# tanishqkumar/ssd

Measured on AMD Instinct MI355X. Metric: output tokens/sec + p50 TTFT, Llama-3-70B SSD k=7 f=3; mean accepted len, higher is better.
Workload: dtype bf16

## Files before the change

ssd_amd/csrc/common.h:

```cpp
#pragma once
#include <hip/hip_runtime.h>
#include <stdint.h>
#include <stdlib.h>

typedef uint16_t bf16_t;
typedef __attribute__((ext_vector_type(8))) __bf16 bf16x8_t;
typedef __attribute__((ext_vector_type(4))) float f32x4_t;
typedef __attribute__((ext_vector_type(4))) short s16x4_t;
typedef __attribute__((ext_vector_type(4))) uint32_t u32x4_t;
typedef __attribute__((ext_vector_type(2))) uint32_t u32x2_t;
constexpr int SSD_MAX_DEVICES = 16;

#include "ssd_hip.h"
#include "ssd_hip_tune.h"
#include "ssd_hip_quant.h"
#include "ssd_hip_w4a16.h"
#include "ssd_hip_w4zp.h"
#include "ssd_hip_mxfp4.h"

__device__ __forceinline__ float bf2f(uint32_t bits16) { return __uint_as_float(bits16 << 16); }

__device__ __forceinline__ uint32_t f2bf(float f) {
  uint32_t u = __float_as_uint(f);
  if ((u & 0x7fffffffu) > 0x7f800000u) return (u >> 16) | 0x40u;
  u += 0x7fffu + ((u >> 16) & 1u);
  return u >> 16;
}
__device__ __forceinline__ uint32_t pack_bf2(float lo, float hi) { return f2bf(lo) | (f2bf(hi) << 16); }

typedef __attribute__((ext_vector_type(2))) float f32x2_t;
typedef __attribute__((ext_vector_type(2))) __bf16 bf16x2_t;
__device__ __forceinline__ uint32_t pack_bf2_hw(float lo, float hi) {
  return __builtin_bit_cast(uint32_t, __builtin_convertvector(f32x2_t{lo, hi}, bf16x2_t));
// ... 92 lines not shown
```

ssd_amd/csrc/gemm.hip:

```cpp
#include "common.h"

enum { EPI_ROWS = 0, EPI_SILU_FRAG = 1, EPI_ROWS_F32 = 2, EPI_ROWS_ARGMAX = 3 };

struct ArgPart { float v; int i; };
__device__ __forceinline__ ArgPart arg_better(ArgPart a, ArgPart b) {
  return (b.v > a.v || (b.v == a.v && b.i < a.i)) ? b : a;
}

extern "C" int ssd_gemm_splitk(const void* x_frag, const void* w_frag, const void* bias, void* y, int M, int N, int K, int ldy,
                               int splits, int waves, void* workspace, void* counters, void* stream);

template <int MT, int NT>
struct Stage {
  u32x4_t a[NT];
  u32x4_t b[MT];
};

template <int MT, int NT, int EPI, bool DEEP = false>
__global__ void __launch_bounds__(DEEP ? 512 : 1024)
gemm_wf_kernel(const u32x4_t* __restrict__ Wf, const u32x4_t* __restrict__ Xf,
               const bf16_t* __restrict__ bias, void* __restrict__ Yv, int M, int N, int K, int ldy, int tpw,
               float* __restrict__ part_val, int* __restrict__ part_idx, int part_stride) {
  extern __shared__ __attribute__((aligned(16))) char smem[];
  constexpr int KTS = EPI == EPI_SILU_FRAG ? 8 : 9;
  KTRACE(KTS, 0);
  const int lane = threadIdx.x & 63;
  const int wave = __builtin_amdgcn_readfirstlane(threadIdx.x >> 6);
  const int nw = blockDim.x >> 6;
  const int KT = K >> 5;
  const int ntiles = (N / 16) / NT;
  const int t_begin = blockIdx.x * tpw, t_end = min(ntiles, t_begin + tpw);
  const u32x4_t* xp = Xf + lane;
  const size_t wstride = (size_t)KT << 6;
  const size_t xstride = (size_t)KT << 6;
  constexpr int U = ((MT + NT <= 3) ? 4 : ((MT + NT <= 6) ? 2 : 1)) * (DEEP ? 2 : 1);
  Stage<MT, NT> cur[U], nxt[U];
  const int kstep = nw * U;
  const int kt0 = wave * U;
// ... 2 lines not shown
  const int mt_last = (M - 1) >> 4;
  auto load = [&](Stage<MT, NT>(&s)[U], int kt) {
#pragma unroll
    for (int u = 0; u < U; ++u) {
#pragma unroll
      for (int nt = 0; nt < NT; ++nt)
        s[u].a[nt] = __builtin_nontemporal_load(wp + nt * wstride + ((size_t)(kt + u) << 6));
#pragma unroll
      for (int mt = 0; mt < MT; ++mt) {
        u32x4_t b = {0u, 0u, 0u, 0u};
        if (NT > 1 || mt * 16 + (lane & 15) < M) b = xp[(mt < mt_last ? mt : mt_last) * xstride + ((size_t)(kt + u) << 6)];
        s[u].b[mt] = b;
      }
    }
  };
  if (t_begin < t_end && kt0 < kmain) load(cur, kt0);
  ArgPart run[MT];
#pragma unroll
  for (int mt = 0; mt < MT; ++mt) run[mt] = ArgPart{-INFINITY, 0x7fffffff};

  for (int tile = t_begin; tile < t_end; ++tile) {
  const int tile0 = tile * NT;
  f32x4_t acc[NT][MT];
#pragma unroll
  for (int nt = 0; nt < NT; ++nt)
#pragma unroll
    for (int mt = 0; mt < MT; ++mt) acc[nt][mt] = f32x4_t{0.f, 0.f, 0.f, 0.f};

  auto compute = [&](Stage<MT, NT>(&s)[U]) {
#pragma unroll
    for (int u = 0; u < U; ++u)
#pragma unroll
      for (int nt = 0; nt < NT; ++nt)
#pragma unroll
        for (int mt = 0; mt < MT; ++mt) acc[nt][mt] = mfma16(s[u].a[nt], s[u].b[mt], acc[nt][mt]);
  };

  int kt = kt0;
  if (kt < kmain) {
    for (; kt + kstep < kmain; kt += kstep) {
      load(nxt, kt + kstep);
      compute(cur);
#pragma unroll
      for (int u = 0; u < U; ++u) cur[u] = nxt[u];
    }
    compute(cur);
  }
  for (kt = (wave == nw - 1) ? kmain : KT; kt < KT; ++kt) {
#pragma unroll
    for (int nt = 0; nt < NT; ++nt) {
      u32x4_t a = __builtin_nontemporal_load(wp + nt * wstride + ((size_t)kt << 6));
#pragma unroll
      for (int mt = 0; mt < MT; ++mt) {
        u32x4_t b = {0u, 0u, 0u, 0u};
        if (mt * 16 + (lane & 15) < M) b = xp[mt * xstride + ((size_t)kt << 6)];
        acc[nt][mt] = mfma16(a, b, acc[nt][mt]);
// ... 102 lines not shown
static int launch_t(const void* x, const void* w, const void* bias, void* y, int M, int N, int K, int ldy,
                    int waves, int tpw, hipStream_t st, float* part_val = nullptr, int* part_idx = nullptr, int part_stride = 0) {
  const int ntiles = (N / 16) / NT;
  if (tpw < 1) tpw = 1;
  const int blocks = (ntiles + tpw - 1) / tpw;
  if (EPI == EPI_ROWS_ARGMAX && (!part_val || !part_idx || part_stride < blocks)) return SSD_ERR_ARG;
  size_t lds = (size_t)waves * NT * MT * 64 * sizeof(f32x4_t);
  if (EPI == EPI_ROWS_ARGMAX) lds += (size_t)waves * MT * 16 * sizeof(ArgPart);
  if (DEEP && waves > 8) return SSD_ERR_ARG;
  auto kern = gemm_wf_kernel<MT, NT, EPI, DEEP>;
  if (lds > 64 * 1024) {
    if (hipFuncSetAttribute(reinterpret_cast<const void*>(kern), hipFuncAttributeMaxDynamicSharedMemorySize, (int)lds) != hipSuccess)
      return SSD_ERR_LAUNCH;
  }
  hipLaunchKernelGGL(kern, dim3(blocks), dim3(waves * 64), lds, st, (const u32x4_t*)w, (const u32x4_t*)x,
                     (const bf16_t*)bias, y, M, N, K, ldy, tpw, part_val, part_idx, part_stride);
  return hipGetLastError() == hipSuccess ? SSD_OK : SSD_ERR_LAUNCH;
}

template <int MT, int EPI>
static int launch_nt(const void* x, const void* w, const void* bias, void* y, int M, int N, int K, int ldy,
                     int nt, int waves, int tpw, hipStream_t st) {
  if (nt == 1) {
    if constexpr (EPI == EPI_SILU_FRAG) return SSD_ERR_ARG;
    else return launch_t<MT, 1, EPI>(x, w, bias, y, M, N, K, ldy, waves, tpw, st);
  }
  if (nt == 2) return launch_t<MT, 2, EPI>(x, w, bias, y, M, N, K, ldy, waves, tpw, st);
  if (nt == 4) {
    if constexpr (MT > 2) return SSD_ERR_ARG;
    else return launch_t<MT, 4, EPI>(x, w, bias, y, M, N, K, ldy, waves, tpw, st);
  }
// ... 63 lines not shown
  }
  int nt = 1;
  if (epilogue == EPI_SILU_FRAG) nt = 2;
  else if (mt >= 4 && groups % 2 == 0) nt = 2;
  else if (groups >= 2048 && groups % 2 == 0) nt = 2;
  int waves = 16;
  while (waves > 1 && KT / waves < 4) waves >>= 1;
  const int blocks = groups / nt;
  if (blocks >= 1024 && waves > 8) waves = 8;
  if (mt == 2 && blocks >= 512 && blocks < 2048 && waves > 4 && KT / 4 >= 4) waves = 4;
  if (mt >= 4 && waves > 8) waves = 8;
  if (mt >= 8 && waves > 4) waves = 4;
  return ssd_gemm_wf_cfg(x_frag, w_frag, bias, y, M, N, K, ldy, epilogue, nt, waves, stream);
}


static void argmax_head_cfg(int M, int N, int K, int* nt, int* waves, int* tpw) {
  const int groups = N / 16, KT = K / 32;
  if (M <= 16) {
    ssd_pick_skinny_cfg(groups, KT, false, nt, waves, tpw);
    return;
  }
  int n = (groups >= 2048 && groups % 2 == 0) ? 2 : 1;
  int w = 16;
  while (w > 1 && KT / w < 4) w >>= 1;
  const int blocks = groups / n;
  if (blocks >= 1024 && w > 8) w = 8;
  if (blocks >= 512 && blocks < 2048 && w > 4 && KT / 4 >= 4) w = 4;
  *nt = n; *waves = w; *tpw = 1;
}
// ... 28 lines not shown
```

ssd_amd/csrc/gemm_fused.hip:

```cpp
#include "common.h"
#include <type_traits>

enum { FEPI_ROWS = 0, FEPI_SILU_FRAG = 1, FEPI_QKV_ROPE = 3 };

struct FusedParams {
  const u32x4_t* Wf;
  const u32x4_t* Xf;
  const bf16_t* h;
  const float* h_parts;
  int S;
  const bf16_t* res_in;
  bf16_t* res_out;
  const bf16_t* norm_w;
  const bf16_t* bias;
  void* y;
  const int64_t* positions;
  const float* cos_sin;
  const int32_t* slots;
  bf16_t* q_out;
  bf16_t* k_cache;
  bf16_t* v_cache;
  float eps;
  int M, N, K, ldy;
  int nh, nkv, hd, bs;
// ... 14 lines not shown
    }
#pragma unroll
    for (int j = 0; j < 4; ++j) { hf[j] = round_bf(lo[j]); hf[4 + j] = round_bf(hi[j]); }
  } else {
    const u32x4_t hv = *reinterpret_cast<const u32x4_t*>(p.h + (size_t)mm * p.K + k8 * 8);
#pragma unroll
    for (int j = 0; j < 4; ++j) { hf[2 * j] = bf2f(hv[j] & 0xffffu); hf[2 * j + 1] = bf2f(hv[j] >> 16); }
  }
#pragma unroll
  for (int j = 0; j < 4; ++j) {
    x[2 * j] = hf[2 * j] + bf2f(rv[j] & 0xffffu);
    x[2 * j + 1] = hf[2 * j + 1] + bf2f(rv[j] >> 16);
  }
}

template <int NT, int EPI, bool XNORM, int FUSED_MAXC>
__global__ void __launch_bounds__(1024) gemm_fused_kernel(const FusedParams p) {
  extern __shared__ __attribute__((aligned(16))) char smem[];
  constexpr int KTS = !XNORM ? 2 : (EPI == FEPI_QKV_ROPE ? 0 : 1);
  KTRACE(KTS, 0);
  const int lane = threadIdx.x & 63;
  const int wave = __builtin_amdgcn_readfirstlane(threadIdx.x >> 6);
  const int nw = blockDim.x >> 6;
  const int M = p.M, K = p.K;
  const int KT = K >> 5, K8 = K >> 3;
  const int tile0 = blockIdx.x * NT;
  const int mcol = lane & 15, q4 = lane >> 4;
  u32x4_t* xlds = reinterpret_cast<u32x4_t*>(smem + p.scratch_bytes);

  f32x4_t acc[NT];
#pragma unroll
  for (int nt = 0; nt < NT; ++nt) acc[nt] = f32x4_t{0.f, 0.f, 0.f, 0.f};
  const u32x4_t* wp = p.Wf + ((size_t)tile0 * KT << 6) + lane;
// ... 3 lines not shown
  u32x4_t wa[2][U][NT];
  u32x4_t xg[2][U];
  auto loadw = [&](int buf, int kt) {
#pragma unroll
    for (int u = 0; u < U; ++u) {
#pragma unroll
      for (int nt = 0; nt < NT; ++nt)
        wa[buf][u][nt] = __builtin_nontemporal_load(wp + nt * wstride + ((size_t)(kt + u) << 6));
      if (!XNORM) {
        u32x4_t b = {0u, 0u, 0u, 0u};
        if (mcol < M) b = p.Xf[((size_t)(kt + u) << 6) + lane];
        xg[buf][u] = b;
      }
    }
  };
  const int kstep = nw * U;
  const int kt0 = wave * U;
  const int ngroups = KT / U;
  const int nmain = ngroups > wave ? (ngroups - wave + nw - 1) / nw : 0;
  if (nmain > 0) loadw(0, kt0);
  if (nmain > 1) loadw(1, kt0 + kstep);
  float pre_cs[8];
  int pre_slot = -1;
  bool pre_ok = false;
  if (EPI == FEPI_QKV_ROPE && wave < NT && mcol < M) {
    const int grp = tile0 + wave;
    const int gph = p.hd >> 4;
    pre_slot = p.slots[mcol];
    if (grp < (p.nh + p.nkv) * gph) {
      const int d = (grp % gph) * 8 + (q4 & 1) * 4;
      const float* cs = p.cos_sin + (size_t)p.positions[mcol] * p.hd;
      const f32x4_t c4 = *reinterpret_cast<const f32x4_t*>(cs + d), s4 = *reinterpret_cast<const f32x4_t*>(cs + (p.hd >> 1) + d);
#pragma unroll
      for (int r = 0; r < 4; ++r) { pre_cs[r] = c4[r]; pre_cs[4 + r] = s4[r]; }
    }
    pre_ok = true;
  }
  KTRACE(KTS, 1);
  if (XNORM) {
    float* ssbuf = reinterpret_cast<float*>(smem);
    constexpr int MC = FUSED_MAXC > 0 ? FUSED_MAXC : 1;
    float x32[MC][8];
    u32x4_t wv[MC];
    const int total = M * K8;
    const bool cached = FUSED_MAXC > 0 && total <= FUSED_MAXC * (int)blockDim.x;
    const int cpb = (K8 + gridDim.x - 1) / gridDim.x;
    if (!cached) {
      for (int c = threadIdx.x; c < total; c += blockDim.x) {
        const int mm = c / K8, k8 = c % K8;
        float xx[8];
        fused_load_x32(p, mm, k8, xx);
        float ss = 0.f;
        u32x4_t o;
// ... 350 lines not shown
  FusedParams q = p;
  if (XNORM) {
    const size_t chunks = (size_t)p.M * (p.K / 8);
    const size_t need = chunks * 4 + (size_t)waves * 64;
    if (lds < need) lds = (need + 15) & ~(size_t)15;
    q.scratch_bytes = (int)lds;
    lds += chunks * 16;
    if (lds > 160 * 1024) return SSD_ERR_SHAPE;
  } else {
    q.scratch_bytes = (int)lds;
  }
  auto kern = gemm_fused_kernel<NT, EPI, XNORM, MAXC>;
  if (lds > 64 * 1024 &&
      hipFuncSetAttribute(reinterpret_cast<const void*>(kern), hipFuncAttributeMaxDynamicSharedMemorySize, (int)lds) != hipSuccess)
    return SSD_ERR_LAUNCH;
  hipLaunchKernelGGL(kern, dim3(blocks), dim3(waves * 64), lds, st, q);
  return hipGetLastError() == hipSuccess ? SSD_OK : SSD_ERR_LAUNCH;
}

template <int NT, int EPI, bool XNORM>
static int launch_fused(const FusedParams& p, int waves, hipStream_t st) {
  if constexpr (XNORM) {
    if (p.M * (p.K / 8) <= waves * 64) return launch_fused_c<NT, EPI, true, 1>(p, waves, st);
    return launch_fused_c<NT, EPI, true, 0>(p, waves, st);
  } else {
    return launch_fused_c<NT, EPI, false, 1>(p, waves, st);
  }
}

template <int EPI, bool XNORM>
static int launch_fused_nt(const FusedParams& p, int nt, int waves, hipStream_t st) {
// ... 61 lines not shown
                              const int32_t* slots, void* q_out, void* k_cache, void* v_cache, int nh, int nkv, int hd,
                              int block_size, int nt, int waves, void* stream) {
  return fused_impl(x_frag, h_rows, nullptr, 0, res_in, res_out, norm_w, eps, w_frag, bias, M, N, K, epilogue, y, ldy, positions,
                    cos_sin, slots, q_out, k_cache, v_cache, nh, nkv, hd, block_size, nt, waves, stream);
}

extern "C" int ssd_gemm_fused_parts(const void* h_parts, int splits, const void* res_in, void* res_out, const void* norm_w,
                                    float eps, const void* w_frag, const void* bias, int M, int N, int K, int epilogue, void* y,
                                    int ldy, const int64_t* positions, const float* cos_sin, const int32_t* slots, void* q_out,
                                    void* k_cache, void* v_cache, int nh, int nkv, int hd, int block_size, int nt, int waves,
                                    void* stream) {
  return fused_impl(nullptr, nullptr, (const float*)h_parts, splits, res_in, res_out, norm_w, eps, w_frag, bias, M, N, K, epilogue,
                    y, ldy, positions, cos_sin, slots, q_out, k_cache, v_cache, nh, nkv, hd, block_size, nt, waves, stream);
}

KT_DEFINE_SETTER(gemm_fused)
```

ssd_amd/engine/model_runner.py:

```python
from __future__ import annotations

import torch
import torch.distributed as dist

from ssd_amd.hip import ops as H
from ssd_amd.hip.lib import load_library
from ssd_amd.model import HipDecoder, AttnMeta
from ssd_amd.model_config import ModelConfig
from ssd_amd import weights as W
from ssd_amd.utils.graphs import capture
from ssd_amd.engine.async_proto import to_device


class ModelRunner:
    PREFILL_GRAPHS = 4
    PREFILL_GRAPH_MAX_T = 1024

    def __init__(self, config, model_cfg: ModelConfig, *, is_draft: bool, device: torch.device, tp_rank: int = 0,
                 tp_size: int = 1, tp_group=None, model_path: str | None = None, weights_seed: int = 0,
                 gen_device: str | None = None, num_kvcache_blocks: int = -1, memory_utilization: float | None = None,
                 max_decode_tokens: int | None = None, weight_source=None, force_collectives: bool = False,
                 custom_ar: bool | None = None):
        if not torch.cuda.is_available():
            raise RuntimeError("ssd_amd.ModelRunner needs an MI355X; there is no CPU fallback on the product path")
# ... 137 lines not shown
        self.sx = self.config.sampler_x
        self.sx_k = (self.config.async_fan_out + 1) if self.sx is not None else 0
        if self.sx is not None:
            rows = max(B * K, self.max_bs * getattr(self.config, "MQ_LEN", 1))
            self.d_boost = torch.zeros(rows, self.sx_k, dtype=torch.int32, **dev)

    def _check_collectives(self) -> None:
        ar = self.model.custom_ar
        if ar is not None and ar.failed():
            raise RuntimeError("one-shot all-reduce timed out waiting for a peer; results of this step are invalid "
                               "(rerun with SSD_CUSTOM_AR=0 to use RCCL)")
        if self._has_chain_err() and (int(self._chain_err_host[0]) or int(self.model.chain_err.item())):
            self._raise_chain_err()

    def _has_chain_err(self) -> bool:
        return getattr(self.model, "chain_seg", False) or getattr(self.model, "tree_seg", False)

    def _raise_chain_err(self):
        raise RuntimeError("a bounded wait inside a resident layer segment (csrc/chain.hip / csrc/tree_segment.hip) gave up; the draft "
                           "forwards since the last check are invalid (rerun with SSD_CHAIN_SEG=0 SSD_TREE_SEG=0 for the separate launches)")

    def _post_chain_err(self) -> None:
        if self._has_chain_err():
            self._chain_err_host.copy_(self.model.chain_err, non_blocking=True)

    def _check_chain_host(self) -> None:
        if self._has_chain_err() and int(self._chain_err_host[0]):
            self._raise_chain_err()

    def check_segments(self, sync: bool = False) -> None:
        if not self._has_chain_err():
            return
        if int(self._chain_err_host[0]) or (sync and int(self.model.chain_err.item())):
            self._raise_chain_err()

# ... 593 lines not shown
```

ssd_amd/model.py:

```python
from __future__ import annotations

from dataclasses import dataclass

import os

import torch
import torch.distributed as dist

from ssd_amd.hip import ops as H
from ssd_amd.hip import quant_ops as Q
from ssd_amd.hip import w4_ops as W4
from ssd_amd.hip import w4zp_ops as W4Z
from ssd_amd.hip import mx4_ops as MX4
from ssd_amd import quant
from ssd_amd.model_config import ModelConfig

BF16 = torch.bfloat16


@dataclass
class AttnMeta:
    mode: int
    B: int
    max_q: int
    slot_mapping: torch.Tensor
    context_lens: torch.Tensor
    block_tables: torch.Tensor
    cu_q: torch.Tensor | None = None
# ... 86 lines not shown
        _validated = _geo == (2048, 2048, 8192, 3072, 64)
        self.chain_seg = ((_cs == "1" or (_cs == "auto" and _validated)) and not cfg.qk_norm and tp_size == 1 and not self.use_coll and not self.quantized
                          and taps is None and H.chain_segment_ok(self.h, self.qn, self.I, self.qkv_n, self.nh, self.nkv, self.hd))
        _ts = os.environ.get("SSD_TREE_SEG", "auto")
        self.tree_seg_rows = 32 if _ts == "1" else 16
        self.tree_seg_colocated = False
        self.tree_seg = ((_ts == "1" or (_ts == "auto" and _validated)) and tp_size == 1 and not self.use_coll and not self.quantized
                         and taps is None and max_tokens >= 2
                         and H.tree_segment_ok(2, self.h, self.qn, self.I, self.qkv_n, self.nh, self.nkv, self.hd))
        if self.chain_seg:
            self.chain_gr = z(H.chain_granule_bytes(self.h, self.I) // 8, dtype=torch.int64)
            self.buf_res3 = z(1, self.h)
        if self.chain_seg or self.tree_seg:
            self.chain_gen = z(1, dtype=torch.int32)
            self.chain_err = z(1, dtype=torch.int32)
        if self.tree_seg:
            self.tree_ws = z(H.tree_segment_workspace_bytes(self.h, self.I) // 8, dtype=torch.int64)
            self.buf_res_b = z(min(T, 32), self.h)
        self._last_parts = False
        pt = min(T, 32)
        self.buf_parts_o = z(16 * pt * self.h, dtype=torch.float32) if self.use_parts else None
        self.buf_parts_d = z(16 * pt * self.h, dtype=torch.float32) if self.use_parts else None
        self.logits = z(self.max_logit_rows, self.V)
        self.taps = sorted(set(taps)) if taps else None
        self.acts = z(T, len(self.taps) * self.h) if self.taps else None
        self.max_splits = 16
        pf_shapes = [(self.qkv_n, self.h), (self.h, self.qn), (2 * self.I, self.h), (self.h, self.I), (self.V, self.h)]
        need = max([H.gemm_pf_workspace_bytes(128, n, k) // 4 for n, k in pf_shapes if self._pf_eligible(n, k)], default=0)
        self._lm_ok = max_tokens > 128
        if self._lm_ok:
# ... 380 lines not shown
                   parts: bool | None = None, pf_src: int = 0) -> None:
        cfg, w = self.cfg, self.w
        p = f"model.layers.{li}."
        small, norm_fuse = self.fusion_plan(T)
        kc, vc = self.kv_cache[li, 0], self.kv_cache[li, 1]
        rope = dict(positions=positions, cos_sin=self.cos_sin, slots=slot_mapping, q_out=self.buf_q, k_cache=kc, v_cache=vc,
                    nh=self.nh, nkv=self.nkv, hd=self.hd, block_size=self.block_size)
        h, res, xf = self.buf_h, self.buf_res, self.buf_xf
        parts = (self.parts_plan(T) if parts is None else parts) and li > 0
        if norm_fuse:
            src = dict(h_parts=self.buf_parts_d, splits=self._parts("d", T)[0]) if parts else dict(h_rows=h)
            H.gemm_fused(w[p + "self_attn.qkv_proj.weight"], T, self.qkv_n, self.h, H.FEPI_QKV_ROPE,
                         res_in=None if li == 0 else res, res_out=self.buf_res2, norm_w=w[p + "input_layernorm.weight"],
                         eps=cfg.rms_norm_eps, bias=w.get(p + "self_attn.qkv_proj.bias"), waves=16, **src, **rope)
            return
        if not gemm_only and not pre_normed:
            if pf_src:
                H.rmsnorm_parts(self._ws_pf, pf_src, T, w[p + "input_layernorm.weight"], cfg.rms_norm_eps, T, self.h,
                                res_in=res, res_out=res, out_frag=xf)
            elif parts:
                H.rmsnorm_parts(self.buf_parts_d, self._parts("d", T)[0], T, w[p + "input_layernorm.weight"], cfg.rms_norm_eps, T, self.h,
                                res_in=res, res_out=res, out_frag=xf)
            else:
                H.rmsnorm(h, w[p + "input_layernorm.weight"], cfg.rms_norm_eps, T, self.h, res_in=None if li == 0 else res,
                          res_out=res, out_frag=xf)
        if small or (16 < T <= 32 and not cfg.qk_norm and not self.quantized):
            H.gemm_fused(w[p + "self_attn.qkv_proj.weight"], T, self.qkv_n, self.h, H.FEPI_QKV_ROPE, x_frag=xf,
                         bias=w.get(p + "self_attn.qkv_proj.bias"), **rope)
        elif (not gemm_only and w.get(p + "self_attn.qkv_proj.bias") is None and self._pf_partials_ok(T, self.qkv_n, self.h)
              and self._pf_splits(T, self.qkv_n, self.h) > 1):
# ... 16 lines not shown
        ws = self.w.get(f"model.layers.{li}.self_attn.o_proj.weight_scale")
        if pf_partials and self._pf_partials_ok(T, self.h, self.qn):
            return self._gemm_pf_partials(self.buf_af, self.qn, w, self.h, T)
        if self.parts_plan(T) if parts is None else parts:
            S, wv = self._parts("o", T)
            H.gemm_parts(self.buf_af, w, T, self.h, self.qn, parts=self.buf_parts_o, splits=S, waves=wv)
        else:
            self._gemm(self.buf_af, self.qn, w, self.h, self.buf_h, T, self.h, scale=ws,
                       zero=self.w.get(f"model.layers.{li}.self_attn.o_proj.weight_zero"))
        return 0

    def launch_gate_up(self, li: int, T: int, gemm_only: bool = False, pre_normed: bool = False, parts: bool | None = None,
                       o_splits: int | None = None, pf_src: int = 0) -> None:
        cfg, w = self.cfg, self.w
        p = f"model.layers.{li}."
        _, norm_fuse = self.fusion_plan(T)
        parts = self.parts_plan(T) if parts is None else parts
        So = o_splits if o_splits is not None else (self._parts("o", T)[0] if parts else 1)
        if norm_fuse:
            src = dict(h_parts=self.buf_parts_o, splits=So) if parts else dict(h_rows=self.buf_h)
            H.gemm_fused(w[p + "mlp.gate_up_proj.weight"], T, 2 * self.I, self.h, H.FEPI_SILU_FRAG,
                         res_in=self.buf_res2, res_out=self.buf_res, norm_w=w[p + "post_attention_layernorm.weight"],
                         eps=cfg.rms_norm_eps, y=self.buf_actf, waves=8, **src)
        else:
            if not gemm_only and not pre_normed:
                if pf_src:
                    H.rmsnorm_parts(self._ws_pf, pf_src, T, w[p + "post_attention_layernorm.weight"], cfg.rms_norm_eps,
                                    T, self.h, res_in=self.buf_res, res_out=self.buf_res, out_frag=self.buf_xf)
                elif parts:
                    H.rmsnorm_parts(self.buf_parts_o, So, T, w[p + "post_attention_layernorm.weight"], cfg.rms_norm_eps,
                                    T, self.h, res_in=self.buf_res, res_out=self.buf_res, out_frag=self.buf_xf)
                else:
                    H.rmsnorm(self.buf_h, w[p + "post_attention_layernorm.weight"], cfg.rms_norm_eps, T, self.h,
                              res_in=self.buf_res, res_out=self.buf_res, out_frag=self.buf_xf)
            self._gemm(self.buf_xf, self.h, w[p + "mlp.gate_up_proj.weight"], 2 * self.I, self.buf_actf, T, 0, epi=H.EPI_SILU_FRAG,
                       scale=w.get(p + "mlp.gate_up_proj.weight_scale"), zero=w.get(p + "mlp.gate_up_proj.weight_zero"))

    def launch_down(self, li: int, T: int, parts: bool | None = None, pf_partials: bool = False) -> int:
# ... 151 lines not shown
```

Before: 114.0.

## Fold RMSNorm into QKV and gate_up GEMMs via in-kernel producer/consumer hand-off

New measurement: 111.6. -2.1%, worse.

```diff
diff --git a/include/ssd_hip_handoff.h b/include/ssd_hip_handoff.h
--- /dev/null
+++ b/include/ssd_hip_handoff.h
@@ -0,0 +1,24 @@
+#ifndef SSD_HIP_HANDOFF_H
+#define SSD_HIP_HANDOFF_H
+#include "ssd_hip.h"
+#ifdef __cplusplus
+extern "C" {
+#endif
+
+int ssd_handoff_state_bytes(void);
+
+int ssd_gemm_fused_handoff(const void* h_rows, const void* res_in, void* res_out, const void* norm_w, float eps, void* x_frag,
+                           const void* w_frag, const void* bias, int M, int N, int K, const int64_t* positions,
+                           const float* cos_sin, const int32_t* slots, void* q_out, void* k_cache, void* v_cache, int nh,
+                           int nkv, int hd, int block_size, void* state, void* err, void* stream);
+int ssd_gemm_fused_handoff_grid(int N, int K);
+
+int ssd_gemm_wf_handoff(const void* h_rows, const void* res_in, void* res_out, const void* norm_w, float eps, void* x_frag,
+                        const void* w_frag, const void* bias, void* y_frag, int M, int N, int K, void* state, void* err,
+                        void* stream);
+int ssd_gemm_wf_handoff_grid(int N, int K);
+
+#ifdef __cplusplus
+}
+#endif
+#endif
diff --git a/profiles/handoff_probe.py b/profiles/handoff_probe.py
--- /dev/null
+++ b/profiles/handoff_probe.py
@@ -0,0 +1,113 @@
+from __future__ import annotations
+
+import argparse
+import json
+import os
+import statistics
+import sys
+
+import torch
+
+sys.path.insert(0, os.path.dirname(os.path.dirname(os.path.abspath(__file__))))
+
+SHAPES = {
+    "70b": (8192, 64, 8, 128, 28672, 80),
+    "8b": (4096, 32, 8, 128, 14336, 32),
+}
+BF = torch.bfloat16
+
+
+def timed(graph, reps):
+    e0, e1 = torch.cuda.Event(enable_timing=True), torch.cuda.Event(enable_timing=True)
+    torch.cuda.synchronize()
+    e0.record()
+    for _ in range(reps):
+        graph.replay()
+    e1.record()
+    torch.cuda.synchronize()
+    return e0.elapsed_time(e1) * 1e3 / reps
+
+
+def main():
+    ap = argparse.ArgumentParser()
+    ap.add_argument("--shape", default="70b", choices=sorted(SHAPES))
+    ap.add_argument("--rows", type=int, nargs="+", default=[8, 7])
+    ap.add_argument("--layers", type=int, default=0)
+    ap.add_argument("--rounds", type=int, default=5)
+    ap.add_argument("--out", default="")
+    a = ap.parse_args()
+    from ssd_amd.hip import ops as H
+    from ssd_amd.hip import handoff_ops as HO
+    h, nh, nkv, hd, I, L = SHAPES[a.shape]
+    L = a.layers or L
+    qkv_n, bs = (nh + 2 * nkv) * hd, 16
+    dev = torch.device("cuda", 0)
+
+    def rnd(*shape, std=0.02):
+        return torch.empty(*shape, dtype=BF, device=dev).normal_(0, std)
+
+    wq = [rnd(qkv_n * h) for _ in range(L)]
+    wg = [rnd(2 * I * h) for _ in range(L)]
+    ln = (1 + rnd(h, std=0.1))
+    cos_sin = torch.rand(512, hd, dtype=torch.float32, device=dev)
+    state, err = HO.handoff_state(dev), torch.zeros(1, dtype=torch.int32, device=dev)
+    lines = []
+    for M in a.rows:
+        hrows, res = rnd(M, h, std=1.0), rnd(M, h, std=1.0)
+        xf = torch.zeros(H.frag_numel(M, h), dtype=BF, device=dev)
+        actf = torch.zeros(H.frag_numel(M, I), dtype=BF, device=dev)
+        q = torch.zeros(M, nh * hd, dtype=BF, device=dev)
+        kc = torch.zeros(2, nkv, bs, hd, dtype=BF, device=dev)
+        vc = torch.zeros_like(kc)
+        rope = dict(positions=torch.arange(M, dtype=torch.int64, device=dev), cos_sin=cos_sin,
+                    slots=torch.full((M,), -1, dtype=torch.int32, device=dev), q_out=q, k_cache=kc, v_cache=vc, nh=nh, nkv=nkv, hd=hd,
+                    block_size=bs)
+
+        def qkv_sep(li):
+            H.rmsnorm(hrows, ln, 1e-5, M, h, res_in=res, res_out=res, out_frag=xf)
+            H.gemm_fused(wq[li], M, qkv_n, h, H.FEPI_QKV_ROPE, x_frag=xf, **rope)
+
+        def qkv_fold(li):
+            HO.gemm_fused_handoff(hrows, ln, 1e-5, xf, wq[li], M, qkv_n, h, state, err, res_in=res, res_out=res, **rope)
+
+        def gu_sep(li):
+            H.rmsnorm(hrows, ln, 1e-5, M, h, res_in=res, res_out=res, out_frag=xf)
+            H.gemm(xf, wg[li], actf, M, 2 * I, h, 0, epilogue=H.EPI_SILU_FRAG)
+
+        def gu_fold(li):
+            HO.gemm_wf_handoff(hrows, ln, 1e-5, xf, wg[li], actf, M, 2 * I, h, state, err, res_in=res, res_out=res)
+
+        for kind, sep, fold in (("norm+qkv", qkv_sep, qkv_fold), ("norm+gate_up", gu_sep, gu_fold)):
+            graphs = {}
+            for name, fn in (("separate", sep), ("folded", fold)):
+                res.normal_(0, 1.0)
+                fn(0)
+                torch.cuda.synchronize()
+                g = torch.cuda.CUDAGraph()
+                with torch.cuda.graph(g):
+                    for li in range(L):
+                        fn(li)
+                g.replay()
+                graphs[name] = g
+            reps = max(2, 128 // L)
+            t = {"separate": [], "folded": []}
+            for _ in range(a.rounds):
+                for name in ("separate", "folded"):
+                    res.normal_(0, 1.0)
+                    t[name].append(timed(graphs[name], reps) / L)
+            med = {k: statistics.median(v) for k, v in t.items()}
+            line = {"probe": "handoff", "shape": a.shape, "kind": kind, "M": M, "layers": L,
+                    "separate_us": round(med["separate"], 2), "folded_us": round(med["folded"], 2),
+                    "saved_us": round(med["separate"] - med["folded"], 2),
+                    "separate_rounds_us": [round(x, 2) for x in t["separate"]], "folded_rounds_us": [round(x, 2) for x in t["folded"]],
+                    "err_word": int(err.item())}
+            print(json.dumps(line), flush=True)
+            lines.append(line)
+    if a.out:
+        with open(a.out, "a") as f:
+            for line in lines:
+                f.write(json.dumps(line) + "\n")
+
+
+if __name__ == "__main__":
+    main()
diff --git a/ssd_amd/csrc/common.h b/ssd_amd/csrc/common.h
--- a/ssd_amd/csrc/common.h
+++ b/ssd_amd/csrc/common.h
@@ -17,6 +17,7 @@
 #include "ssd_hip_w4a16.h"
 #include "ssd_hip_w4zp.h"
 #include "ssd_hip_mxfp4.h"
+#include "ssd_hip_handoff.h"
 
 __device__ __forceinline__ float bf2f(uint32_t bits16) { return __uint_as_float(bits16 << 16); }
 
diff --git a/ssd_amd/csrc/gemm.hip b/ssd_amd/csrc/gemm.hip
--- a/ssd_amd/csrc/gemm.hip
+++ b/ssd_amd/csrc/gemm.hip
@@ -1,4 +1,5 @@
 #include "common.h"
+#include "handoff.h"
 
 enum { EPI_ROWS = 0, EPI_SILU_FRAG = 1, EPI_ROWS_F32 = 2, EPI_ROWS_ARGMAX = 3 };
 
@@ -16,12 +17,15 @@
   u32x4_t b[MT];
 };
 
-template <int MT, int NT, int EPI, bool DEEP = false>
+typedef const u32x4_t* __restrict__ xf_restrict_t;
+template <int MT, int NT, int EPI, bool DEEP = false, bool HO = false>
 __global__ void __launch_bounds__(DEEP ? 512 : 1024)
-gemm_wf_kernel(const u32x4_t* __restrict__ Wf, const u32x4_t* __restrict__ Xf,
+gemm_wf_kernel(const u32x4_t* __restrict__ Wf, std::conditional_t<HO, const u32x4_t*, xf_restrict_t> Xf,
                const bf16_t* __restrict__ bias, void* __restrict__ Yv, int M, int N, int K, int ldy, int tpw,
-               float* __restrict__ part_val, int* __restrict__ part_idx, int part_stride) {
+               float* __restrict__ part_val, int* __restrict__ part_idx, int part_stride, const HandoffParams ho) {
   extern __shared__ __attribute__((aligned(16))) char smem[];
+  const unsigned ho_grid = HO ? __builtin_amdgcn_readfirstlane(gridDim.x) : 0u;
+  if (HO) ho_draw_ticket(ho, ho_grid, K, smem);
   constexpr int KTS = EPI == EPI_SILU_FRAG ? 8 : 9;
   KTRACE(KTS, 0);
   const int lane = threadIdx.x & 63;
@@ -54,7 +58,36 @@
       }
     }
   };
-  if (t_begin < t_end && kt0 < kmain) load(cur, kt0);
+  auto load_w = [&](Stage<MT, NT>(&s)[U], int kt) {
+#pragma unroll
+    for (int u = 0; u < U; ++u)
+#pragma unroll
+      for (int nt = 0; nt < NT; ++nt)
+        s[u].a[nt] = __builtin_nontemporal_load(wp + nt * wstride + ((size_t)(kt + u) << 6));
+  };
+  auto load_x = [&](Stage<MT, NT>(&s)[U], int kt) {
+#pragma unroll
+    for (int u = 0; u < U; ++u)
+#pragma unroll
+      for (int mt = 0; mt < MT; ++mt) {
+        u32x4_t b = {0u, 0u, 0u, 0u};
+        if (NT > 1 || mt * 16 + (lane & 15) < M) b = xp[(mt < mt_last ? mt : mt_last) * xstride + ((size_t)(kt + u) << 6)];
+        s[u].b[mt] = b;
+      }
+  };
+  bool pre2 = false;
+  if (HO) {
+    const bool first = t_begin < t_end && kt0 < kmain;
+    pre2 = DEEP && first && kt0 + kstep < kmain;
+    if (first) load_w(cur, kt0);
+    const ho_u64 tag = ho_produce(ho, ho_grid, M, K, smem);
+    if (pre2) load_w(nxt, kt0 + kstep);
+    ho_wait(ho, tag, M);
+    if (first) load_x(cur, kt0);
+    if (pre2) load_x(nxt, kt0 + kstep);
+  } else {
+    if (t_begin < t_end && kt0 < kmain) load(cur, kt0);
+  }
   ArgPart run[MT];
 #pragma unroll
   for (int mt = 0; mt < MT; ++mt) run[mt] = ArgPart{-INFINITY, 0x7fffffff};
@@ -79,7 +112,8 @@
   int kt = kt0;
   if (kt < kmain) {
     for (; kt + kstep < kmain; kt += kstep) {
-      load(nxt, kt + kstep);
+      if (!(HO && pre2)) load(nxt, kt + kstep);
+      pre2 = false;
       compute(cur);
 #pragma unroll
       for (int u = 0; u < U; ++u) cur[u] = nxt[u];
@@ -212,7 +246,7 @@
       return SSD_ERR_LAUNCH;
   }
   hipLaunchKernelGGL(kern, dim3(blocks), dim3(waves * 64), lds, st, (const u32x4_t*)w, (const u32x4_t*)x,
-                     (const bf16_t*)bias, y, M, N, K, ldy, tpw, part_val, part_idx, part_stride);
+                     (const bf16_t*)bias, y, M, N, K, ldy, tpw, part_val, part_idx, part_stride, HandoffParams{});
   return hipGetLastError() == hipSuccess ? SSD_OK : SSD_ERR_LAUNCH;
 }
 
@@ -306,6 +340,55 @@
   return ssd_gemm_wf_cfg(x_frag, w_frag, bias, y, M, N, K, ldy, epilogue, nt, waves, stream);
 }
 
+static bool handoff_silu_cfg(int N, int K, int* nt, int* waves, int* tpw, bool* deep) {
+  if ((N & 31) || (K & 31) || N <= 0 || K <= 0 || K > 16384) return false;
+  const int groups = N / 16, KT = K / 32;
+  ssd_pick_skinny_cfg(groups, KT, true, nt, waves, tpw);
+  if (groups % *nt) return false;
+  *deep = g_deep_mode && *waves == 8 && KT >= 256 && *nt == 4 && groups % 512 == 0 && groups / 512 <= 8;
+  return true;
+}
+
+extern "C" int ssd_gemm_wf_handoff_grid(int N, int K) {
+  int nt, waves, tpw; bool deep;
+  if (!handoff_silu_cfg(N, K, &nt, &waves, &tpw, &deep)) return SSD_ERR_SHAPE;
+  const int ntiles = (N / 16) / nt;
+  return (ntiles + tpw - 1) / tpw;
+}
+
+template <int NT, bool DEEP>
+static int launch_handoff(const void* w, const void* bias, void* y, int M, int N, int K, int waves, int tpw, const HandoffParams& ho,
+                          hipStream_t st) {
+  const int ntiles = (N / 16) / NT;
+  const int blocks = (ntiles + tpw - 1) / tpw;
+  size_t lds = (size_t)waves * NT * 64 * sizeof(f32x4_t);
+  if (lds < ho_lds_bytes(K)) lds = (ho_lds_bytes(K) + 15) & ~(size_t)15;
+  auto kern = gemm_wf_kernel<1, NT, EPI_SILU_FRAG, DEEP, true>;
+  if (lds > 64 * 1024 &&
+      hipFuncSetAttribute(reinterpret_cast<const void*>(kern), hipFuncAttributeMaxDynamicSharedMemorySize, (int)lds) != hipSuccess)
+    return SSD_ERR_LAUNCH;
+  hipLaunchKernelGGL(kern, dim3(blocks), dim3(waves * 64), lds, st, (const u32x4_t*)w, (const u32x4_t*)ho.xf, (const bf16_t*)bias, y, M, N,
+                     K, 0, tpw, (float*)nullptr, (int*)nullptr, 0, ho);
+  return hipGetLastError() == hipSuccess ? SSD_OK : SSD_ERR_LAUNCH;
+}
+
+extern "C" int ssd_gemm_wf_handoff(const void* h_rows, const void* res_in, void* res_out, const void* norm_w, float eps, void* x_frag,
+                                   const void* w_frag, const void* bias, void* y_frag, int M, int N, int K, void* state, void* err,
+                                   void* stream) {
+  if (M <= 0 || M > 16) return SSD_ERR_SHAPE;
+  int nt, waves, tpw; bool deep;
+  if (!handoff_silu_cfg(N, K, &nt, &waves, &tpw, &deep)) return SSD_ERR_SHAPE;
+  if (!h_rows || !norm_w || !x_frag || !w_frag || !y_frag || !state || !err) return SSD_ERR_ARG;
+  HandoffParams ho;
+  ho.h = (const bf16_t*)h_rows; ho.res_in = (const bf16_t*)res_in; ho.res_out = (bf16_t*)res_out; ho.norm_w = (const bf16_t*)norm_w;
+  ho.xf = (u32x4_t*)x_frag; ho.state = (ho_u64*)state; ho.err = (unsigned*)err; ho.eps = eps; ho.spin_budget = HO_SPIN_BUDGET;
+  hipStream_t st = (hipStream_t)stream;
+  if (deep) return launch_handoff<4, true>(w_frag, bias, y_frag, M, N, K, waves, tpw, ho, st);
+  if (nt == 2) return launch_handoff<2, false>(w_frag, bias, y_frag, M, N, K, waves, tpw, ho, st);
+  return launch_handoff<4, false>(w_frag, bias, y_frag, M, N, K, waves, tpw, ho, st);
+}
+
+extern "C" int ssd_handoff_state_bytes(void) { return HO_STATE_WORDS * 8; }
 
 static void argmax_head_cfg(int M, int N, int K, int* nt, int* waves, int* tpw) {
   const int groups = N / 16, KT = K / 32;
diff --git a/ssd_amd/csrc/gemm_fused.hip b/ssd_amd/csrc/gemm_fused.hip
--- a/ssd_amd/csrc/gemm_fused.hip
+++ b/ssd_amd/csrc/gemm_fused.hip
@@ -1,4 +1,5 @@
 #include "common.h"
+#include "handoff.h"
 #include <type_traits>
 
 enum { FEPI_ROWS = 0, FEPI_SILU_FRAG = 1, FEPI_QKV_ROPE = 3 };
@@ -52,9 +53,12 @@
   }
 }
 
-template <int NT, int EPI, bool XNORM, int FUSED_MAXC>
-__global__ void __launch_bounds__(1024) gemm_fused_kernel(const FusedParams p) {
+template <int NT, int EPI, bool XNORM, int FUSED_MAXC, bool HO = false>
+__global__ void __launch_bounds__(1024) gemm_fused_kernel(const FusedParams p, const HandoffParams ho) {
   extern __shared__ __attribute__((aligned(16))) char smem[];
+  static_assert(!(HO && XNORM), "the hand-off form takes fragment-major x");
+  const unsigned ho_grid = HO ? __builtin_amdgcn_readfirstlane(gridDim.x) : 0u;
+  if (HO) ho_draw_ticket(ho, ho_grid, p.K, smem);
   constexpr int KTS = !XNORM ? 2 : (EPI == FEPI_QKV_ROPE ? 0 : 1);
   KTRACE(KTS, 0);
   const int lane = threadIdx.x & 63;
@@ -88,12 +92,34 @@
       }
     }
   };
+  auto loadwt = [&](int buf, int kt) {
+#pragma unroll
+    for (int u = 0; u < U; ++u)
+#pragma unroll
+      for (int nt = 0; nt < NT; ++nt)
+        wa[buf][u][nt] = __builtin_nontemporal_load(wp + nt * wstride + ((size_t)(kt + u) << 6));
+  };
+  auto loadx = [&](int buf, int kt) {
+#pragma unroll
+    for (int u = 0; u < U; ++u) {
+      u32x4_t b = {0u, 0u, 0u, 0u};
+      if (mcol < M) b = p.Xf[((size_t)(kt + u) << 6) + lane];
+      xg[buf][u] = b;
+    }
+  };
   const int kstep = nw * U;
   const int kt0 = wave * U;
   const int ngroups = KT / U;
   const int nmain = ngroups > wave ? (ngroups - wave + nw - 1) / nw : 0;
-  if (nmain > 0) loadw(0, kt0);
-  if (nmain > 1) loadw(1, kt0 + kstep);
+  ho_u64 tag = 0;
+  if (HO) {
+    if (nmain > 0) loadwt(0, kt0);
+    tag = ho_produce(ho, ho_grid, M, K, smem);
+    if (nmain > 1) loadwt(1, kt0 + kstep);
+  } else {
+    if (nmain > 0) loadw(0, kt0);
+    if (nmain > 1) loadw(1, kt0 + kstep);
+  }
   float pre_cs[8];
   int pre_slot = -1;
   bool pre_ok = false;
@@ -111,6 +137,11 @@
     pre_ok = true;
   }
   KTRACE(KTS, 1);
+  if (HO) {
+    ho_wait(ho, tag, M);
+    if (nmain > 0) loadx(0, kt0);
+    if (nmain > 1) loadx(1, kt0 + kstep);
+  }
   if (XNORM) {
     float* ssbuf = reinterpret_cast<float*>(smem);
     constexpr int MC = FUSED_MAXC > 0 ? FUSED_MAXC : 1;
@@ -491,7 +522,7 @@
   if (lds > 64 * 1024 &&
       hipFuncSetAttribute(reinterpret_cast<const void*>(kern), hipFuncAttributeMaxDynamicSharedMemorySize, (int)lds) != hipSuccess)
     return SSD_ERR_LAUNCH;
-  hipLaunchKernelGGL(kern, dim3(blocks), dim3(waves * 64), lds, st, q);
+  hipLaunchKernelGGL(kern, dim3(blocks), dim3(waves * 64), lds, st, q, HandoffParams{});
   return hipGetLastError() == hipSuccess ? SSD_OK : SSD_ERR_LAUNCH;
 }
 
@@ -583,4 +614,57 @@
                     y, ldy, positions, cos_sin, slots, q_out, k_cache, v_cache, nh, nkv, hd, block_size, nt, waves, stream);
 }
 
+static bool handoff_qkv_cfg(int N, int K, int* nt, int* waves) {
+  if ((N & 15) || (K & 31) || N <= 0 || K <= 0 || K > 16384) return false;
+  int tpw;
+  ssd_pick_skinny_cfg(N / 16, K / 32, false, nt, waves, &tpw);
+  return *waves <= 16 && (N / 16) % *nt == 0 && *nt != 2;
+}
+
+extern "C" int ssd_gemm_fused_handoff_grid(int N, int K) {
+  int nt, waves;
+  if (!handoff_qkv_cfg(N, K, &nt, &waves)) return SSD_ERR_SHAPE;
+  return (N / 16) / nt;
+}
+
+template <int NT>
+static int launch_fused_handoff(const FusedParams& p, const HandoffParams& ho, int waves, hipStream_t st) {
+  size_t lds = (size_t)waves * NT * 64 * sizeof(f32x4_t);
+  if (lds < ho_lds_bytes(p.K)) lds = (ho_lds_bytes(p.K) + 15) & ~(size_t)15;
+  FusedParams q = p;
+  q.scratch_bytes = (int)lds;
+  auto kern = gemm_fused_kernel<NT, FEPI_QKV_ROPE, false, 1, true>;
+  if (lds > 64 * 1024 &&
+      hipFuncSetAttribute(reinterpret_cast<const void*>(kern), hipFuncAttributeMaxDynamicSharedMemorySize, (int)lds) != hipSuccess)
+    return SSD_ERR_LAUNCH;
+  hipLaunchKernelGGL(kern, dim3((p.N / 16) / NT), dim3(waves * 64), lds, st, q, ho);
+  return hipGetLastError() == hipSuccess ? SSD_OK : SSD_ERR_LAUNCH;
+}
+
+extern "C" int ssd_gemm_fused_handoff(const void* h_rows, const void* res_in, void* res_out, const void* norm_w, float eps, void* x_frag,
+                                      const void* w_frag, const void* bias, int M, int N, int K, const int64_t* positions,
+                                      const float* cos_sin, const int32_t* slots, void* q_out, void* k_cache, void* v_cache, int nh,
+                                      int nkv, int hd, int block_size, void* state, void* err, void* stream) {
+  if (M <= 0 || M > 16) return SSD_ERR_SHAPE;
+  int nt, waves;
+  if (!handoff_qkv_cfg(N, K, &nt, &waves)) return SSD_ERR_SHAPE;
+  if (hd != 64 && hd != 128 && hd != 256) return SSD_ERR_SHAPE;
+  if (N != (nh + 2 * nkv) * hd || block_size <= 0) return SSD_ERR_SHAPE;
+  if (!h_rows || !norm_w || !x_frag || !w_frag || !state || !err) return SSD_ERR_ARG;
+  if (!positions || !cos_sin || !slots || !q_out || !k_cache || !v_cache) return SSD_ERR_ARG;
+  FusedParams p;
+  p.Wf = (const u32x4_t*)w_frag; p.Xf = (const u32x4_t*)x_frag; p.h = nullptr; p.h_parts = nullptr; p.S = 0;
+  p.res_in = nullptr; p.res_out = nullptr; p.norm_w = nullptr;
+  p.bias = (const bf16_t*)bias; p.y = nullptr; p.positions = positions; p.cos_sin = cos_sin; p.slots = slots;
+  p.q_out = (bf16_t*)q_out; p.k_cache = (bf16_t*)k_cache; p.v_cache = (bf16_t*)v_cache;
+  p.eps = eps; p.M = M; p.N = N; p.K = K; p.ldy = 0; p.nh = nh; p.nkv = nkv; p.hd = hd; p.bs = block_size; p.scratch_bytes = 0;
+  HandoffParams ho;
+  ho.h = (const bf16_t*)h_rows; ho.res_in = (const bf16_t*)res_in; ho.res_out = (bf16_t*)res_out; ho.norm_w = (const bf16_t*)norm_w;
+  ho.xf = (u32x4_t*)x_frag; ho.state = (ho_u64*)state; ho.err = (unsigned*)err; ho.eps = eps; ho.spin_budget = HO_SPIN_BUDGET;
+  hipStream_t st = (hipStream_t)stream;
+  if (nt == 1) return launch_fused_handoff<1>(p, ho, waves, st);
+  if (nt == 4) return launch_fused_handoff<4>(p, ho, waves, st);
+  return SSD_ERR_ARG;
+}
+
 KT_DEFINE_SETTER(gemm_fused)
diff --git a/ssd_amd/csrc/handoff.h b/ssd_amd/csrc/handoff.h
--- /dev/null
+++ b/ssd_amd/csrc/handoff.h
@@ -0,0 +1,137 @@
+#pragma once
+#include "common.h"
+#include <type_traits>
+
+typedef unsigned long long ho_u64;
+#define HO_AGENT __HIP_MEMORY_SCOPE_AGENT
+constexpr int HO_STATE_WORDS = 24;
+constexpr int HO_FLAG0 = 8;
+constexpr int HO_COUNT_BITS = 24;
+constexpr long HO_SPIN_BUDGET = 200000L;
+
+struct HandoffParams {
+  const bf16_t* h;
+  const bf16_t* res_in;
+  bf16_t* res_out;
+  const bf16_t* norm_w;
+  u32x4_t* xf;
+  ho_u64* state;
+  unsigned* err;
+  float eps;
+  long spin_budget;
+};
+
+static inline size_t ho_lds_bytes(int K) { return (size_t)K * 4 + 64 + 16; }
+
+__device__ __forceinline__ void ho_barrier_lds() { asm volatile("s_waitcnt lgkmcnt(0)\n\ts_barrier" ::: "memory"); }
+
+__device__ __forceinline__ void ho_draw_ticket(const HandoffParams& p, unsigned G, int K, char* lds) {
+  if (threadIdx.x == 0) {
+    const ho_u64 t = __hip_atomic_fetch_add(p.state, 1ull, __ATOMIC_RELAXED, HO_AGENT);
+    *reinterpret_cast<ho_u64*>(lds + (size_t)K * 4 + 64) = t;
+    if ((unsigned)(t & ((1ull << HO_COUNT_BITS) - 1)) == G - 1)
+      __hip_atomic_fetch_add(p.state, (1ull << HO_COUNT_BITS) - (ho_u64)G, __ATOMIC_RELAXED, HO_AGENT);
+  }
+}
+
+__device__ __forceinline__ void ho_norm_row(const HandoffParams& p, int row, int K, float* vrow, float* red) {
+  const int H8 = K >> 3, KT = K >> 5;
+  const int VT = K >= 4096 ? 1024 : 256;
+  const u32x4_t* x = reinterpret_cast<const u32x4_t*>(p.h) + (size_t)row * H8;
+  const u32x4_t* rin = p.res_in ? reinterpret_cast<const u32x4_t*>(p.res_in) + (size_t)row * H8 : nullptr;
+  u32x4_t* rout = p.res_out ? reinterpret_cast<u32x4_t*>(p.res_out) + (size_t)row * H8 : nullptr;
+  for (int vt = threadIdx.x; vt < VT; vt += blockDim.x) {
+    float ss = 0.f;
+#pragma unroll 1
+    for (int i = 0; i < 2; ++i) {
+      const int c = vt + i * VT;
+      if (c < H8) {
+        const u32x4_t xv = x[c];
+        u32x4_t rv = {0u, 0u, 0u, 0u};
+        if (rin) rv = rin[c];
+        u32x4_t ro;
+        float v[8];
+#pragma unroll
+        for (int j = 0; j < 4; ++j) {
+          float lo = bf2f(xv[j] & 0xffffu), hi = bf2f(xv[j] >> 16);
+          if (rin) { lo += bf2f(rv[j] & 0xffffu); hi += bf2f(rv[j] >> 16); }
+          v[2 * j] = lo; v[2 * j + 1] = hi;
+          ro[j] = pack_bf2(lo, hi);
+          ss += lo * lo; ss += hi * hi;
+        }
+        if (rout) rout[c] = ro;
+        *reinterpret_cast<f32x4_t*>(vrow + c * 8) = f32x4_t{v[0], v[1], v[2], v[3]};
+        *reinterpret_cast<f32x4_t*>(vrow + c * 8 + 4) = f32x4_t{v[4], v[5], v[6], v[7]};
+      }
+    }
+    ss = wave_sum(ss);
+    if ((threadIdx.x & 63) == 0) red[vt >> 6] = ss;
+  }
+  ho_barrier_lds();
+  float tot = 0.f;
+  const int nred = VT >> 6;
+  for (int i = 0; i < nred; ++i) tot += red[i];
+  const float rs = 1.0f / sqrtf(tot / (float)K + p.eps);
+  const u32x4_t* w = reinterpret_cast<const u32x4_t*>(p.norm_w);
+  for (int vt = threadIdx.x; vt < VT; vt += blockDim.x) {
+#pragma unroll 1
+    for (int i = 0; i < 2; ++i) {
+      const int c = vt + i * VT;
+      if (c < H8) {
+        const u32x4_t wv = w[c];
+        const f32x4_t a = *reinterpret_cast<const f32x4_t*>(vrow + c * 8), b = *reinterpret_cast<const f32x4_t*>(vrow + c * 8 + 4);
+        const float v[8] = {a[0], a[1], a[2], a[3], b[0], b[1], b[2], b[3]};
+        u32x4_t o;
+#pragma unroll
+        for (int j = 0; j < 4; ++j) {
+          const float lo = (v[2 * j] * rs) * bf2f(wv[j] & 0xffffu);
+          const float hi = (v[2 * j + 1] * rs) * bf2f(wv[j] >> 16);
+          o[j] = pack_bf2(lo, hi);
+        }
+        p.xf[frag_chunk(row, c, KT)] = o;
+      }
+    }
+  }
+  ho_barrier_lds();
+}
+
+__device__ __forceinline__ ho_u64 ho_produce(const HandoffParams& p, unsigned G, int M, int K, char* lds) {
+  float* vrow = reinterpret_cast<float*>(lds);
+  float* red = vrow + K;
+  const ho_u64* bc = reinterpret_cast<const ho_u64*>(red + 16);
+  ho_barrier_lds();
+  const ho_u64 t = *bc;
+  const unsigned lt = (unsigned)(t & ((1ull << HO_COUNT_BITS) - 1));
+  const ho_u64 tag = (t >> HO_COUNT_BITS) + 1;
+  const unsigned P = G < (unsigned)M ? G : (unsigned)M;
+  if (lt < P) {
+    for (int row = (int)lt; row < M; row += (int)P) ho_norm_row(p, row, K, vrow, red);
+    asm volatile("s_waitcnt vmcnt(0)" ::: "memory");
+    __syncthreads();
+    if (threadIdx.x == 0) {
+      __builtin_amdgcn_fence(__ATOMIC_RELEASE, "agent");
+      asm volatile("s_waitcnt vmcnt(0)" ::: "memory");
+      for (int row = (int)lt; row < M; row += (int)P) __hip_atomic_store(p.state + HO_FLAG0 + row, tag, __ATOMIC_RELAXED, HO_AGENT);
+    }
+  }
+  return tag;
+}
+
+constexpr unsigned HO_ERR_GAVE_UP = 1u;
+
+__device__ __forceinline__ void ho_wait(const HandoffParams& p, ho_u64 tag, int M) {
+  if (threadIdx.x < 64) {
+    const int lane = threadIdx.x;
+    long spins = 0;
+    for (;;) {
+      ho_u64 v = tag;
+      if (lane < M) v = __hip_atomic_load(p.state + HO_FLAG0 + lane, __ATOMIC_RELAXED, HO_AGENT);
+      if (__ballot(v == tag) == ~0ull) break;
+      if (++spins > p.spin_budget) { if (lane == 0) atomicExch(p.err, HO_ERR_GAVE_UP); break; }
+      __builtin_amdgcn_s_sleep(2);
+    }
+    __builtin_amdgcn_fence(__ATOMIC_ACQUIRE, "agent");
+    asm volatile("s_waitcnt vmcnt(0)" ::: "memory");
+  }
+  ho_barrier_lds();
+}
diff --git a/ssd_amd/engine/model_runner.py b/ssd_amd/engine/model_runner.py
--- a/ssd_amd/engine/model_runner.py
+++ b/ssd_amd/engine/model_runner.py
@@ -175,11 +175,12 @@
             self._raise_chain_err()
 
     def _has_chain_err(self) -> bool:
-        return getattr(self.model, "chain_seg", False) or getattr(self.model, "tree_seg", False)
+        return getattr(self.model, "chain_seg", False) or getattr(self.model, "tree_seg", False) or getattr(self.model, "handoff", False)
 
     def _raise_chain_err(self):
-        raise RuntimeError("a bounded wait inside a resident layer segment (csrc/chain.hip / csrc/tree_segment.hip) gave up; the draft "
-                           "forwards since the last check are invalid (rerun with SSD_CHAIN_SEG=0 SSD_TREE_SEG=0 for the separate launches)")
+        raise RuntimeError("a bounded wait inside a resident layer segment (csrc/chain.hip / csrc/tree_segment.hip) or a hand-off GEMM "
+                           "(csrc/handoff.h) gave up; the forwards since the last check are invalid (rerun with SSD_CHAIN_SEG=0 "
+                           "SSD_TREE_SEG=0 SSD_HANDOFF=0 for the separate launches)")
 
     def _post_chain_err(self) -> None:
         if self._has_chain_err():
diff --git a/ssd_amd/hip/handoff_ops.py b/ssd_amd/hip/handoff_ops.py
--- /dev/null
+++ b/ssd_amd/hip/handoff_ops.py
@@ -0,0 +1,77 @@
+from __future__ import annotations
+
+import ctypes as C
+
+import torch
+
+from .lib import load_library, SsdHipError
+from .ops import _p, _stream, _check
+
+c_void_p, c_int, c_float = C.c_void_p, C.c_int, C.c_float
+
+HANDOFF_SIGNATURES = {
+    "ssd_handoff_state_bytes": [],
+    "ssd_gemm_fused_handoff": [c_void_p, c_void_p, c_void_p, c_void_p, c_float, c_void_p, c_void_p, c_void_p, c_int, c_int, c_int,
+                               c_void_p, c_void_p, c_void_p, c_void_p, c_void_p, c_void_p, c_int, c_int, c_int, c_int, c_void_p,
+                               c_void_p, c_void_p],
+    "ssd_gemm_fused_handoff_grid": [c_int, c_int],
+    "ssd_gemm_wf_handoff": [c_void_p, c_void_p, c_void_p, c_void_p, c_float, c_void_p, c_void_p, c_void_p, c_void_p, c_int, c_int,
+                            c_int, c_void_p, c_void_p, c_void_p],
+    "ssd_gemm_wf_handoff_grid": [c_int, c_int],
+}
+
+_HOLIB = None
+
+
+def load_handoff_library():
+    global _HOLIB
+    if _HOLIB is not None:
+        return _HOLIB
+    lib = load_library()
+    for name, args in HANDOFF_SIGNATURES.items():
+        try:
+            fn = getattr(lib, name)
+        except AttributeError as e:
+            raise SsdHipError(f"libssdhip.so does not export {name}") from e
+        fn.argtypes = args
+        fn.restype = c_int
+    _HOLIB = lib
+    return lib
+
+
+def handoff_state(device) -> torch.Tensor:
+    return torch.zeros(load_handoff_library().ssd_handoff_state_bytes() // 8, dtype=torch.int64, device=device)
+
+
+def qkv_handoff_grid(N: int, K: int) -> int:
+    return load_handoff_library().ssd_gemm_fused_handoff_grid(N, K)
+
+
+def gate_up_handoff_grid(N: int, K: int) -> int:
+    return load_handoff_library().ssd_gemm_wf_handoff_grid(N, K)
+
+
+def gemm_fused_handoff(h_rows, norm_w, eps: float, x_frag, w_frag, M: int, N: int, K: int, state, err, *, res_in=None, res_out=None,
+                       bias=None, positions=None, cos_sin=None, slots=None, q_out=None, k_cache=None, v_cache=None, nh: int = 0,
+                       nkv: int = 0, hd: int = 0, block_size: int = 0):
+    _check(load_handoff_library().ssd_gemm_fused_handoff(_p(h_rows), _p(res_in), _p(res_out), _p(norm_w), eps, _p(x_frag), _p(w_frag),
+                                                         _p(bias), M, N, K, _p(positions), _p(cos_sin), _p(slots), _p(q_out),
+                                                         _p(k_cache), _p(v_cache), nh, nkv, hd, block_size, _p(state), _p(err),
+                                                         _stream()), "ssd_gemm_fused_handoff")
+
+
+def gemm_wf_handoff(h_rows, norm_w, eps: float, x_frag, w_frag, y_frag, M: int, N: int, K: int, state, err, *, res_in=None,
+                    res_out=None, bias=None):
+    _check(load_handoff_library().ssd_gemm_wf_handoff(_p(h_rows), _p(res_in), _p(res_out), _p(norm_w), eps, _p(x_frag), _p(w_frag),
+                                                      _p(bias), _p(y_frag), M, N, K, _p(state), _p(err), _stream()),
+           "ssd_gemm_wf_handoff")
+
+
+def give_up_message() -> str:
+    return ("a bounded wait inside a hand-off GEMM (csrc/handoff.h) gave up; the forwards since the last check are invalid "
+            "(rerun with SSD_HANDOFF=0 for the separate launches)")
+
+
+def check_error_word(word: int) -> None:
+    if int(word):
+        raise RuntimeError(give_up_message())
diff --git a/ssd_amd/model.py b/ssd_amd/model.py
--- a/ssd_amd/model.py
+++ b/ssd_amd/model.py
@@ -12,6 +12,7 @@
 from ssd_amd.hip import w4_ops as W4
 from ssd_amd.hip import w4zp_ops as W4Z
 from ssd_amd.hip import mx4_ops as MX4
+from ssd_amd.hip import handoff_ops as HO
 from ssd_amd import quant
 from ssd_amd.model_config import ModelConfig
 
@@ -128,6 +129,15 @@
         if self.chain_seg or self.tree_seg:
             self.chain_gen = z(1, dtype=torch.int32)
             self.chain_err = z(1, dtype=torch.int32)
+        self.handoff = (os.environ.get("SSD_HANDOFF", "1") != "0" and not self.quantized and not self.use_coll and not cfg.qk_norm
+                        and tp_size == 1 and device.type == "cuda")
+        self.ho_qkv = self.handoff and HO.qkv_handoff_grid(self.qkv_n, self.h) > 0
+        self.ho_gu = self.handoff and HO.gate_up_handoff_grid(2 * self.I, self.h) > 0
+        self.handoff = self.ho_qkv or self.ho_gu
+        if self.handoff:
+            self.ho_state = HO.handoff_state(device)
+            if not (self.chain_seg or self.tree_seg):
+                self.chain_err = z(1, dtype=torch.int32)
         if self.tree_seg:
             self.tree_ws = z(H.tree_segment_workspace_bytes(self.h, self.I) // 8, dtype=torch.int64)
             self.buf_res_b = z(min(T, 32), self.h)
@@ -538,6 +548,11 @@
                          res_in=None if li == 0 else res, res_out=self.buf_res2, norm_w=w[p + "input_layernorm.weight"],
                          eps=cfg.rms_norm_eps, bias=w.get(p + "self_attn.qkv_proj.bias"), waves=16, **src, **rope)
             return
+        if self.ho_qkv and small and not (gemm_only or pre_normed or pf_src or parts):
+            HO.gemm_fused_handoff(h, w[p + "input_layernorm.weight"], cfg.rms_norm_eps, xf, w[p + "self_attn.qkv_proj.weight"], T,
+                                  self.qkv_n, self.h, self.ho_state, self.chain_err, res_in=None if li == 0 else res, res_out=res,
+                                  bias=w.get(p + "self_attn.qkv_proj.bias"), **rope)
+            return
         if not gemm_only and not pre_normed:
             if pf_src:
                 H.rmsnorm_parts(self._ws_pf, pf_src, T, w[p + "input_layernorm.weight"], cfg.rms_norm_eps, T, self.h,
@@ -584,7 +599,7 @@
                        o_splits: int | None = None, pf_src: int = 0) -> None:
         cfg, w = self.cfg, self.w
         p = f"model.layers.{li}."
-        _, norm_fuse = self.fusion_plan(T)
+        small, norm_fuse = self.fusion_plan(T)
         parts = self.parts_plan(T) if parts is None else parts
         So = o_splits if o_splits is not None else (self._parts("o", T)[0] if parts else 1)
         if norm_fuse:
@@ -592,6 +607,10 @@
             H.gemm_fused(w[p + "mlp.gate_up_proj.weight"], T, 2 * self.I, self.h, H.FEPI_SILU_FRAG,
                          res_in=self.buf_res2, res_out=self.buf_res, norm_w=w[p + "post_attention_layernorm.weight"],
                          eps=cfg.rms_norm_eps, y=self.buf_actf, waves=8, **src)
+        elif self.ho_gu and small and not (gemm_only or pre_normed or pf_src or parts):
+            HO.gemm_wf_handoff(self.buf_h, w[p + "post_attention_layernorm.weight"], cfg.rms_norm_eps, self.buf_xf,
+                               w[p + "mlp.gate_up_proj.weight"], self.buf_actf, T, 2 * self.I, self.h, self.ho_state, self.chain_err,
+                               res_in=self.buf_res, res_out=self.buf_res)
         else:
             if not gemm_only and not pre_normed:
                 if pf_src:
```
